# rpl-cmu/bevrender

Measured on AMD Instinct MI355X. Metric: samples/sec fwd+bwd, 6-cam 256x704 BEV-lift+corr, higher is better.
Workload: dtype bf16; 1 GPU; cfg3: 6-cam 256x704 features (64x64x176), 200x200 BEV, C=64 h=2 D=5, L=2 encoder layers (TSA+SCA), T=2 (1 no-grad history frame(s) + 1 fwd+bwd), correlation head with contrastive + lifted-structure losses, AdamW; batch 8 per GPU; backbone/render CNN excluded; global_batch=8, per_gpu_batch=8, parallelism=dp1

## Files before the change

bevrender_amd/_lib.py:

```python
from __future__ import annotations

import ctypes as C
import os
import subprocess
import threading

import torch

_HERE = os.path.dirname(os.path.abspath(__file__))
LIB_PATH = os.environ.get("BEVRENDER_LIB") or os.path.join(_HERE, "lib", "libbevrender_hip.so")
CSRC = os.path.join(_HERE, "csrc")

PREC_F32, PREC_BF16, PREC_F16, PREC_BF16X3 = 0, 1, 2, 3
ABI_VERSION = 6

SYMBOLS = [
    "bevr_abi_version", "bevr_strerror", "bevr_attn_table_dims", "bevr_attn_key_ws_bytes", "bevr_attn_key_prep",
    "bevr_attn_fwd", "bevr_attn_bwd_q",
    "bevr_attn_bwd_k", "bevr_attn_fwd_dropout", "bevr_attn_bwd_q_dropout", "bevr_attn_bwd_k_dropout", "bevr_attn_cell_fwd", "bevr_attn_cell_bwd_q", "bevr_attn_cell_bwd_k", "bevr_attn_tap_ws_bytes", "bevr_attn_tap_prep", "bevr_attn_tap_fwd", "bevr_attn_tap_bwd_q", "bevr_attn_tap_bwd_k", "bevr_attn_tap_fwd_dropout", "bevr_attn_tap_bwd_q_dropout", "bevr_attn_tap_bwd_k_dropout", "bevr_attn_gather_fwd", "bevr_attn_gather_fwd_rows", "bevr_attn_gather_fwd_x3", "bevr_attn_slab_ws_bytes", "bevr_attn_slab_prep", "bevr_attn_slab_bwd_q", "bevr_attn_slab_rows_ws_bytes", "bevr_attn_slab_rows_prep", "bevr_attn_slab_bwd_q_rows", "bevr_sample_fwd", "bevr_sample_bwd", "bevr_sample_fwd_bf16", "bevr_sample_bwd_bf16", "bevr_project_bev_grid", "bevr_project_bev_grid_masked", "bevr_corr_fwd",
    "bevr_corr_bwd", "bevr_recall_rank", "bevr_dwconv_fwd", "bevr_dwconv_bwd_w", "bevr_dwconv_res_gelu", "bevr_affine_warp_fwd", "bevr_affine_warp_bwd",
    "bevr_attn_bwd_k_ws_bytes", "bevr_attn_bwd_k_ws", "bevr_attn_tap_bwd_k_ws_bytes", "bevr_attn_tap_bwd_k_ws",
    "bevr_attn_slab_x3_ws_bytes", "bevr_attn_slab_x3_prep", "bevr_attn_slab_bwd_q_x3",
    "bevr_attn_tap_fwd_x3_dropout", "bevr_attn_tap_bwd_q_x3_dropout", "bevr_attn_tap_bwd_k_x3_dropout",
    "bevr_offset_head_fwd", "bevr_offset_head_bwd", "bevr_key_positions_fwd", "bevr_key_positions_bwd", "bevr_kv_project", "bevr_layernorm_fwd", "bevr_layernorm_bwd", "bevr_merge_views_fwd", "bevr_merge_views_bwd", "bevr_merge_tap_fwd", "bevr_merge_tap_bwd", "bevr_attn_bwd_prep", "bevr_pack_kv", "bevr_unpack_dkv",
]


class AttnDesc(C.Structure):
    _fields_ = [(n, C.c_int32) for n in (
        "n_prob", "q_div", "heads", "groups", "S", "Sp", "N", "Np", "Ht", "Wt", "Hp", "Wp",
        "y_off", "x_off", "precision", "reserved")]


class BevrError(RuntimeError):
    pass


_lib = None
_lock = threading.Lock()


def build(verbose: bool = False) -> str:
    cmd = ["make", "-C", CSRC, "-j", "4"]
    res = subprocess.run(cmd, capture_output=True, text=True)
    if verbose or res.returncode != 0:
        print(res.stdout)
        print(res.stderr)
# ... 57 lines not shown
        L.bevr_attn_slab_rows_prep.argtypes = [dp, fp, fp, vp, vp, vp]
        L.bevr_attn_slab_bwd_q_rows.argtypes = [dp, vp, vp, vp, vp, fp, vp, fp, fp, fp, fp, fp, ip, ip, vp]
        L.bevr_attn_slab_x3_ws_bytes.argtypes = [dp]
        L.bevr_attn_slab_x3_prep.argtypes = [dp, fp, fp, vp, vp, vp]
        L.bevr_attn_slab_bwd_q_x3.argtypes = [dp, vp, vp, vp, vp, fp, vp, fp, fp, fp, fp, fp, vp]
        L.bevr_sample_fwd.argtypes = [fp, fp, fp] + [ip] * 5 + [vp]
        L.bevr_sample_bwd.argtypes = [fp] * 5 + [ip] * 5 + [vp]
        L.bevr_sample_fwd_bf16.argtypes = [vp, fp, fp] + [ip] * 5 + [vp]
        L.bevr_sample_bwd_bf16.argtypes = [vp] + [fp] * 4 + [ip] * 5 + [vp]
        L.bevr_project_bev_grid.argtypes = [fp] * 4 + [ip] * 4 + [vp]
        L.bevr_project_bev_grid_masked.argtypes = [fp] * 4 + [ip] * 4 + [vp] + [ip] * 3 + [vp]
        L.bevr_corr_fwd.argtypes = [fp] * 5 + [ip] * 4 + [vp]
        L.bevr_corr_bwd.argtypes = [fp] * 8 + [ip] * 4 + [vp]
        L.bevr_recall_rank.argtypes = [fp, vp, ip, vp]
        L.bevr_dwconv_fwd.argtypes = [fp, fp, fp, fp] + [ip] * 7 + [vp]
        L.bevr_dwconv_bwd_w.argtypes = [fp, fp, fp, fp] + [ip] * 6 + [vp]
        L.bevr_dwconv_res_gelu.argtypes = [fp] * 5 + [ip] * 6 + [vp]
        L.bevr_affine_warp_fwd.argtypes = [fp, fp, fp] + [ip] * 4 + [vp]
        L.bevr_affine_warp_bwd.argtypes = [fp, fp, fp] + [ip] * 4 + [vp]
        L.bevr_offset_head_fwd.argtypes = [fp] * 7 + [C.c_longlong] + [ip] * 4 + [C.c_float, vp]
        L.bevr_offset_head_bwd.argtypes = [fp] * 13 + [C.c_longlong] + [ip] * 4 + [C.c_float, vp]
        L.bevr_layernorm_fwd.argtypes = [fp] * 6 + [C.c_longlong, ip, C.c_float, vp]
        L.bevr_layernorm_bwd.argtypes = [fp] * 8 + [C.c_longlong, ip, vp]
        L.bevr_kv_project.argtypes = [vp, ip, fp, C.c_longlong, vp, fp] + [ip] * 9 + [vp] * 6 + [ip, vp]
        L.bevr_key_positions_fwd.argtypes = [fp, fp, vp, fp] + [ip] * 8 + [C.c_float, C.c_float, vp]
        L.bevr_key_positions_bwd.argtypes = [fp, fp, vp, fp, fp] + [ip] * 8 + [C.c_float, C.c_float, vp]
        L.bevr_pack_kv.argtypes = [fp, fp, C.c_longlong, C.c_longlong] + [ip] * 6 + [vp] * 5
        L.bevr_merge_views_fwd.argtypes = [fp] * 5 + [ip] * 6 + [vp]
        L.bevr_merge_views_bwd.argtypes = [fp] * 9 + [ip] * 6 + [vp]
        L.bevr_merge_tap_fwd.argtypes = [fp] * 7 + [ip] * 6 + [vp]
        L.bevr_merge_tap_bwd.argtypes = [fp] * 13 + [ip] * 6 + [vp]
        L.bevr_attn_bwd_prep.argtypes = [fp] * 5 + [vp, vp, fp, fp] + [ip] * 3 + [vp]
        L.bevr_unpack_dkv.argtypes = [fp] * 4 + [C.c_longlong, C.c_longlong] + [ip] * 5 + [vp]
        for name in SYMBOLS:
            fn = getattr(L, name)
            if name in ("bevr_attn_key_ws_bytes", "bevr_attn_tap_ws_bytes", "bevr_attn_slab_ws_bytes",
                        "bevr_attn_slab_rows_ws_bytes", "bevr_attn_slab_x3_ws_bytes", "bevr_attn_bwd_k_ws_bytes", "bevr_attn_tap_bwd_k_ws_bytes"):
                fn.restype = C.c_size_t
            elif name not in ("bevr_strerror",):
                fn.restype = C.c_int
        if L.bevr_abi_version() != ABI_VERSION:
            raise BevrError(f"libbevrender_hip.so ABI version {L.bevr_abi_version()} != {ABI_VERSION}: rebuild "
                            "(make -C bevrender_amd/csrc)")
        _lib = L
    return _lib

# ... 6 lines not shown
```

bevrender_amd/csrc/dwconv.hip:

```cpp
#include "bevr_common.h"

namespace {

struct DwGeom {
  int B, H, W, C, k;
  long sb, sy, sx, sc;
  int nhwc;
};

__global__ __launch_bounds__(256) void dwconv_fwd_kernel(DwGeom g, const float* __restrict__ x, const float* __restrict__ w,
                                                         const float* __restrict__ bias, float* __restrict__ y, int flip) {
  const long n = (long)g.B * g.H * g.W * g.C;
  const long idx = (long)blockIdx.x * 256 + threadIdx.x;
  if (idx >= n) return;
  int c, xx, yy, b;
  if (g.nhwc) { c = idx % g.C; long t = idx / g.C; xx = t % g.W; t /= g.W; yy = t % g.H; b = t / g.H; }
  else { xx = idx % g.W; long t = idx / g.W; yy = t % g.H; t /= g.H; c = t % g.C; b = t / g.C; }
  const int p = g.k / 2;
  const float* wc = w + (long)c * g.k * g.k;
  const float* xb = x + b * g.sb + c * g.sc;
  float acc = bias ? bias[c] : 0.f;
  for (int dy = 0; dy < g.k; ++dy) {
    const int iy = yy + dy - p;
    if (iy < 0 || iy >= g.H) continue;
// ... 232 lines not shown
  }
  const DwGeom g = make_geom(B, H, W, C, k, nhwc);
  const long n = (long)B * H * W * C;
  hipLaunchKernelGGL(dwconv_fwd_kernel, dim3((unsigned)((n + 255) / 256)), dim3(256), 0, (hipStream_t)stream, g, x, w, bias, y,
                     flip);
  return (int)hipGetLastError();
}

extern "C" int bevr_dwconv_res_gelu(const float* x, const float* w, const float* bias, const float* aux, float* y, int B, int H,
                                    int W, int C, int k, int mode, void* stream) {
  if (!x || !w || !y || (mode == 2 && !aux)) return BEVR_E_NULL;
  if (B <= 0 || H <= 0 || W <= 0 || C <= 0 || (C & 3) || k != 3 || mode < 1 || mode > 3) return BEVR_E_SHAPE;
  if (!bevr_aligned16(x) || !bevr_aligned16(y) || (bias && !bevr_aligned16(bias)) || (aux && !bevr_aligned16(aux)))
    return BEVR_E_ALIGN;
  const long nthr = (long)B * H * ((W + DW_XT - 1) / DW_XT) * (C >> 2);
  const dim3 grid((unsigned)((nthr + 255) / 256));
  hipStream_t st = (hipStream_t)stream;
  if (mode == 1)
    hipLaunchKernelGGL((dwconv_fwd_nhwc4_kernel<3, 1>), grid, dim3(256), 0, st, B, H, W, C, x, w, bias, aux, y, 0);
  else if (mode == 2)
    hipLaunchKernelGGL((dwconv_fwd_nhwc4_kernel<3, 2>), grid, dim3(256), 0, st, B, H, W, C, x, w, bias, aux, y, 0);
  else
    hipLaunchKernelGGL((dwconv_fwd_nhwc4_kernel<3, 3>), grid, dim3(256), 0, st, B, H, W, C, x, w, (const float*)nullptr, aux, y, 1);
  return (int)hipGetLastError();
}

constexpr int DW_BANDS = 4;
__global__ __launch_bounds__(256) void dwconv_bwd_w_nchw3_kernel(int H, int W, const float* __restrict__ x,
                                                                const float* __restrict__ dy_, float* __restrict__ dw,
                                                                float* __restrict__ dbias, int C) {
  __shared__ float red[4][10];
  const int plane = blockIdx.x, band = blockIdx.y, xx = threadIdx.x;
  const int c = plane % C;
  const int rows = (H + DW_BANDS - 1) / DW_BANDS, y0 = band * rows, y1 = min(H, y0 + rows);
  const float* xp = x + (size_t)plane * H * W;
  const float* dp = dy_ + (size_t)plane * H * W;
  const bool on = xx < W;
  auto row3 = [&](int yy, float (&r)[3]) {
    const bool ry = on && yy >= 0 && yy < H;
    r[0] = (ry && xx >= 1) ? xp[(size_t)yy * W + xx - 1] : 0.f;
    r[1] = ry ? xp[(size_t)yy * W + xx] : 0.f;
    r[2] = (ry && xx + 1 < W) ? xp[(size_t)yy * W + xx + 1] : 0.f;
  };
  float acc[9] = {0.f, 0.f, 0.f, 0.f, 0.f, 0.f, 0.f, 0.f, 0.f}, accb = 0.f;
  float ra[3], rb[3], rc[3];
  row3(y0 - 1, ra);
// ... 53 lines not shown
```

bevrender_amd/model/SCA.py:

```python
import os

import torch
import torch.nn as nn

from .. import ops
from .SCA_deform_attn import SCADeformableAttention


MIN_CELL_KEYS = int(os.environ.get("BEVR_CELL_MIN", "1024"))


def pillar_grid(bev_bound, S: int, D: int, z_shift: float) -> torch.Tensor:
    X, Y, Z = float(bev_bound["X"]), float(bev_bound["Y"]), float(bev_bound["Z"])
    xs, ys, zs = X / S, Y / S, Z / D

    def bins(start, end, step, n):
        v = torch.arange(start, end, step)
        if v.numel() < n:
            raise ValueError("BEV bound / shape produce too few bins")
        return v[:n]

    gx = bins(0 + xs, X + xs, 2 * xs, S // 2)
    gy = bins(-Y + ys, Y + ys, 2 * ys, S)
    gz = bins(-Z + zs + z_shift, Z + zs + z_shift, 2 * zs, D)
# ... 18 lines not shown
            batch_size=batch_size, n_views=n_views, attn_drop_rate=attn_drop_rate, proj_drop_rate=proj_drop_rate,
            data_type=data_type, logger=logger, precision=precision)

    def sample_3d_points(self) -> torch.Tensor:
        return pillar_grid(self.bev_bound, self.bev_feat_shape, self.bev_depth_dim, self.z_shift)

    @property
    def points_2d_dict(self):
        return self.projector.bev_grid_to_camera(self.sample_3d_points())

    def reference_points(self, vehicle_code: int, device):
        key = (int(vehicle_code), str(device))
        if key not in self._ref_cache:
            pts = self.projector.bev_grid_to_camera(self.sample_3d_points(), device=device)[int(vehicle_code)]
            r = torch.stack(pts, 0)
            V, _, h, w, d = r.shape
            ref = r.permute(0, 2, 3, 4, 1).reshape(V, h, w * d, 2).contiguous()
            S, D = self.bev_feat_shape, self.bev_depth_dim
            yx = ref.reshape(V, -1, 2)[..., (1, 0)].double().cpu().numpy()
            order, split = ops.split_key_order(yx, S, 2 * S * D - 1, MIN_CELL_KEYS)
            self._ref_cache[key] = (ref, order.to(device), split)
        return self._ref_cache[key]

    def forward(self, query, img_feat, vehicle_type_idx, wandb_log_dict, return_wandb_log=True):
        B = query.shape[0]
        code = int(vehicle_type_idx) if not torch.is_tensor(vehicle_type_idx) else self._code(vehicle_type_idx)
        ref, order, split = self.reference_points(code, query.device)
        ref = ref[None].expand(B, -1, -1, -1, -1)
        if img_feat.dim() == 4:
            img_feat = img_feat.reshape(B, self.num_views, *img_feat.shape[1:])
        return self.spatial_deform_attn(x=img_feat, query=query, reference_points=ref,
                                        wandb_log_dict=wandb_log_dict, return_wandb_log=return_wandb_log,
                                        key_order=order, cell_split=split, split_is_pinned=True)

    def _code(self, t: torch.Tensor) -> int:
        codes = self.projector.vehicle_codes()
        if len(codes) == 1:
            return codes[0]
        return int(t.item())
```

bevrender_amd/model/SCA_deform_attn.py:

```python
import os

import torch
import torch.nn.functional as F
from torch import nn

from .. import ops, resolve_precision
from .model_utils import LayerNormProxy, attention_dropout, trunc_normal_

CELL_TAIL = int(os.environ.get("BEVR_CELL_TAIL", "128"))


class SCADeformableAttention(nn.Module):
    def __init__(self, bev_feat_shape, bev_depth_dim, dim_embed, n_heads, n_groups, stride, kernel_size,
                 scale_offset_range, batch_size, n_views=3, attn_drop_rate=0.0, proj_drop_rate=0.0,
                 data_type=torch.float32, logger=None, precision=None):
        super().__init__()
        self.n_channel_per_head = dim_embed // n_heads
        self.scale = self.n_channel_per_head ** -0.5
        self.n_heads = n_heads
        self.embed_dim = self.n_channel_per_head * n_heads
        self.n_groups = n_groups
        self.n_channel_per_group = self.embed_dim // n_groups
        self.n_heads_per_group = n_heads // n_groups
        self.query_height = self.query_width = bev_feat_shape
# ... 56 lines not shown
                rng = off.new_tensor([1.0 / (Hk - 1.0), 1.0 / (Wk - 1.0)]).reshape(1, 2, 1, 1)
                off = off.tanh() * rng * self.offset_range_factor
            pos = off.permute(0, 2, 3, 1).reshape(B, g, Hk, Wk, 2) + ref[:, v, None]
            if not self.scale_offset_range:
                pos = pos.clamp(-1.0, 1.0)
            outs.append(pos.reshape(B, g, Hk * Wk, 2))
        pos = torch.stack(outs, 1)
        if key_order is not None:
            N = Hk * Wk
            pos = pos.gather(3, key_order[None, :, None, :, None].expand(B, V, g, N, 2))
        return pos

    def _pinned_keys_tap(self, S, Hi, Wi):
        if not (self.scale_offset_range and ops.tap_supported(self.precision, self.n_groups)):
            return False
        Hk, Wk = S // 2, S * self.bev_depth_dim
        if Hk < 2 or Wk < 2:
            return False
        ymax = 0.5 * self.offset_range_factor / (Hk - 1.0) * (Hi - 1)
        xmax = 0.5 * self.offset_range_factor / (Wk - 1.0) * (Wi - 1)
        return (ymax < ops.TAP_R - 1 - 1e-3 or Hi <= ops.TAP_R) and (xmax < ops.TAP_C - 1 - 1e-3 or Wi <= ops.TAP_C)

    def forward(self, x, query, reference_points, wandb_log_dict, return_wandb_log=True, key_order=None,
                cell_split=None, split_is_pinned=False):
        B, V, C, Hi, Wi = x.shape
        S = query.shape[-1]
        if V != self.n_views:
            raise ValueError(f"expected {self.n_views} views, got {V}")
        g = self.n_groups
        pos = self.key_positions(query, reference_points.to(query.dtype), key_order)
        N = pos.shape[3]
        pos = pos.reshape(B * V * g, N, 2)
        drop = attention_dropout(self)
        Wt = self.rpe_table.shape[-1]
        pinned = split_is_pinned and self._pinned_keys_tap(S, Hi, Wi)
        if not (cell_split is not None and cell_split < N and g == 1):
            cell_split = None
        source = "kv"
        if x.is_cuda and ops.kv_source_supported(C, self.n_heads, g, self.precision):
            source = "kv_source"
        elif (x.is_cuda and pinned and cell_split is not None and self.precision == ops._lib.PREC_BF16X3
              and (drop is None or ops.tap_supported(self.precision, g, dropout=True))):
            source = "tap_pix"
        tap_source = False
        if cell_split is not None:
            route = ops.attention_route(self.precision, g, S, Wt, N, cell_split, "pinned" if pinned and source != "kv" else False,
                                        drop is not None, source, C, self.n_heads)
# ... 3 lines not shown
            n_tail = min(CELL_TAIL, max(0, N - cell_split - 1024))
            with torch.no_grad():
                a, b = ops.key_coords(pos[:, cell_split:], S, Wt, N - cell_split)
                dyn = ops.cell_order(a, b, n_tail)
            pos = torch.cat((pos[:, :cell_split], pos[:, cell_split:].gather(1, dyn[..., None].expand(-1, -1, 2))), 1)
            cell_split = cell_split + n_tail
        Wkv = torch.cat((self.proj_k.weight.flatten(1), self.proj_v.weight.flatten(1)), 0)
        bkv = torch.cat((self.proj_k.bias, self.proj_v.bias), 0)
        xf = x.reshape(B * V, C, Hi, Wi)
        if source == "kv_source":
            feat = (xf if xf.dtype == torch.bfloat16 else xf.float()).permute(0, 2, 3, 1).contiguous()
            src = dict(kv_source=(feat, Wkv, bkv))
        elif source == "tap_pix":
            xs = ops.sample_features(xf, pos[:, :cell_split].contiguous(), g)
            src = dict(kv=F.linear(xs, Wkv, bkv), tap_pix=(xf.permute(0, 2, 3, 1), Wkv, bkv))
        else:
            xs = ops.sample_features(xf, pos, g)
            src = dict(kv=F.linear(xs, Wkv, bkv))
        o = ops.attention_core(query, None, None, pos, self.rpe_table, heads=self.n_heads, groups=g, views=V,
                               precision=self.precision, cell_split=cell_split, tap_source=tap_source, attn_drop=drop,
                               concat_views=True, **src)
        out = ops.linear_rows(o, self.proj_out.weight.flatten(1), self.proj_out.bias)
        out = F.dropout(out, self.proj_drop_rate, self.training)
        return out.permute(0, 2, 1).reshape(B, C, S, S), wandb_log_dict
```

bevrender_amd/model/TSA.py:

```python
import torch
import torch.nn as nn

from .TSA_deform_attn import TSADeformableAttention


class TemporalSelfAttn(nn.Module):
    def __init__(self, bev_feat_shape, dim_embed, n_heads, n_groups, stride, kernel_size, batch_size,
                 scale_offset_range, n_views=3, attn_drop_rate=0.0, proj_drop_rate=0.0, data_type=torch.float32,
                 logger=None, precision=None):
        super().__init__()
        self.logger = logger
        assert n_heads % n_groups == 0, "n_heads must be divisible by n_groups"
        self.temporal_deform_attn = TSADeformableAttention(
            bev_feat_shape=bev_feat_shape, dim_embed=dim_embed, n_heads=n_heads, n_groups=n_groups, stride=stride,
            kernel_size=kernel_size, scale_offset_range=scale_offset_range, batch_size=batch_size, n_views=n_views,
            attn_drop_rate=attn_drop_rate, proj_drop_rate=proj_drop_rate, data_type=data_type, logger=logger,
            precision=precision)

    def forward(self, query, prev_bev, wandb_log_dict, return_wandb_log=True):
        return self.temporal_deform_attn(x=prev_bev, query=query, wandb_log_dict=wandb_log_dict,
                                         return_wandb_log=return_wandb_log)
```

bevrender_amd/model/TSA_deform_attn.py:

```python
import torch
import torch.nn.functional as F
from torch import nn

from .. import ops, resolve_precision
from .model_utils import (LayerNormProxy, attention_dropout, _dw_ok, depthwise_conv2d, depthwise_conv2d_nhwc, normalized_grid,
                          trunc_normal_)


class TSADeformableAttention(nn.Module):
    def __init__(self, bev_feat_shape, dim_embed, n_heads, n_groups, stride, kernel_size, scale_offset_range,
                 batch_size, n_views=3, attn_drop_rate=0.0, proj_drop_rate=0.0, data_type=torch.float32,
                 logger=None, precision=None):
        super().__init__()
        self.n_channel_per_head = dim_embed // n_heads
        self.scale = self.n_channel_per_head ** -0.5
        self.n_heads = n_heads
        self.embed_dim = self.n_channel_per_head * n_heads
        self.n_groups = n_groups
        self.n_channel_per_group = self.embed_dim // n_groups
        self.n_heads_per_group = n_heads // n_groups
        self.bev_h = self.bev_w = bev_feat_shape
        self.batch_size = batch_size
        self.scale_offset_range = scale_offset_range
        self.kernel_size, self.stride, self.n_views = kernel_size, stride, n_views
# ... 41 lines not shown
                                  co[3].weight.flatten(1), 1, co[1].norm.eps).permute(0, 3, 1, 2)
        else:
            y = co[2](co[1](z))
            off = F.linear(y.permute(0, 2, 3, 1), co[3].weight.flatten(1)).permute(0, 3, 1, 2)
        Hk, Wk = off.shape[-2:]
        if off.is_cuda and Hk > 1 and Wk > 1:
            fac = self.offset_range_factor if self.scale_offset_range else 1.0
            grid = normalized_grid(Hk, Wk, torch.float32, off.device).reshape(1, Hk * Wk, 2)
            pos = ops.key_positions(off.permute(0, 2, 3, 1).reshape(1, B * g, Hk * Wk, 2), grid,
                                    self._key_order(Hk, Wk, off.device)[None], B, g, sca_SD=None,
                                    use_tanh=bool(self.scale_offset_range), sy=fac / (Hk - 1.0), sx=fac / (Wk - 1.0))
            return pos.reshape(B * g, Hk * Wk, 2)
        if self.scale_offset_range:
            rng = off.new_tensor([1.0 / (Hk - 1.0), 1.0 / (Wk - 1.0)]).reshape(1, 2, 1, 1)
            off = off.tanh() * rng * self.offset_range_factor
        pos = off.permute(0, 2, 3, 1) + normalized_grid(Hk, Wk, off.dtype, off.device)[None]
        if not self.scale_offset_range:
            pos = pos.clamp(-1.0, 1.0)
        pos = pos.reshape(B * g, Hk * Wk, 2)
        if Hk > 1 and Wk > 1:
            pos = pos.index_select(1, self._key_order(Hk, Wk, pos.device))
        return pos

    def forward(self, x, query, wandb_log_dict, return_wandb_log=True):
        if x is None:
            x = query
        B, C, H, W = x.shape
        pos = self.key_positions(query)
        Wkv = torch.cat((self.proj_k.weight.flatten(1), self.proj_v.weight.flatten(1)), 0)
        bkv = torch.cat((self.proj_k.bias, self.proj_v.bias), 0)
        drop = attention_dropout(self)
        if x.is_cuda and ops.kv_source_supported(C, self.n_heads, self.n_groups, self.precision):
            feat = (x if x.dtype == torch.bfloat16 else x.float()).permute(0, 2, 3, 1).contiguous()
            o = ops.attention_core(query, None, None, pos, self.rpe_table, heads=self.n_heads, groups=self.n_groups,
                                   views=1, precision=self.precision, kv_source=(feat, Wkv, bkv), attn_drop=drop)
        else:
            xs = ops.sample_features(x, pos, self.n_groups)
            kv = F.linear(xs, Wkv, bkv)
            o = ops.attention_core(query, None, None, pos, self.rpe_table, heads=self.n_heads, groups=self.n_groups,
                                   views=1, precision=self.precision, kv=kv, attn_drop=drop)
        out = ops.linear_rows(o, self.proj_out.weight.flatten(1), self.proj_out.bias)
        out = F.dropout(out, self.proj_drop_rate, self.training)
        out = out.permute(0, 2, 1).reshape(B, C, H, W)
        return out, wandb_log_dict
```

bevrender_amd/model/encoder.py:

```python
import math

import torch
import torch.nn as nn
import torch.nn.functional as F

from .SCA import SpatialCrossAttn
from .TSA import TemporalSelfAttn
from .feedforward import FeedForwardLayer
from .img_backbone import PatchProjection, ResNet18_wo_fpn
from .model_utils import LayerNormProxy, TransformerMLPWithConv, depthwise_conv2d


class DropPath(nn.Module):

    def __init__(self, drop_prob=0.0):
        super().__init__()
        self.drop_prob = drop_prob

    def forward(self, x):
        if self.drop_prob == 0.0 or not self.training:
            return x
        keep = 1.0 - self.drop_prob
        mask = x.new_empty((x.shape[0],) + (1,) * (x.dim() - 1)).bernoulli_(keep)
        return x * mask / keep


class EncoderLayer(nn.Module):
    def __init__(self, bev_bound, bev2cmr_projector, n_views, bev_feat_shape, bev_depth_dim, z_shift, dim_embed,
                 expansion, stage_idx, n_groups, n_heads, stride, kernel_size, batch_size, scale_offset_range,
                 attn_drop_rate=0.0, proj_drop_rate=0.0, mlp_drop_rate=0.0, drop_path_rate=0.2, ffn_drop_rate=0.1,
                 data_type=torch.float32, logger=None, precision=None):
        super().__init__()
        self.logger, self.stage_idx, self.bev_feat_shape = logger, stage_idx, bev_feat_shape
# ... 1 lines not shown
        self.layer_scale = nn.Identity()
        self.layer_norm = LayerNormProxy(C)
        self.tsa_mlp = TransformerMLPWithConv(C, expansion, mlp_drop_rate)
        self.sca_mlp = TransformerMLPWithConv(C, expansion, mlp_drop_rate)
        self.drop_path = DropPath(drop_path_rate) if drop_path_rate > 0.0 else nn.Identity()
        self.tsa_local_percept_unit = nn.Conv2d(C, C, 3, 1, 1, groups=C)
        self.sca_local_percept_unit = nn.Conv2d(C, C, 3, 1, 1, groups=C)
        self.down_proj = nn.Sequential(nn.Conv2d(C, 2 * C, 3, 2, 1, bias=False), LayerNormProxy(2 * C))
        self.ffn_tsa = FeedForwardLayer(in_dim=bev_feat_shape, hidden_dim=C, dropout=ffn_drop_rate)
        self.ffn_sca = FeedForwardLayer(in_dim=bev_feat_shape, hidden_dim=C, dropout=ffn_drop_rate)
        common = dict(bev_feat_shape=bev_feat_shape, dim_embed=C, n_heads=n_heads, n_groups=n_groups, stride=stride,
                      kernel_size=kernel_size, batch_size=batch_size, scale_offset_range=scale_offset_range,
                      n_views=n_views, attn_drop_rate=attn_drop_rate, proj_drop_rate=proj_drop_rate,
                      data_type=data_type, logger=logger, precision=precision)
        self.temporal_self_attn = TemporalSelfAttn(**common)
        self.spatial_cross_attn = SpatialCrossAttn(bev_bound=bev_bound, bev2cmr_projector=bev2cmr_projector,
                                                   bev_depth_dim=bev_depth_dim, z_shift=z_shift, **common)

    def forward(self, bev_query, img_tensor, prev_bev, vehicle_pose, vehicle_type_idx, wandb_log_dict,
                return_wandb_log=True):
        x = bev_query
        if prev_bev is not None and not self.training:
            prev_bev = self.project_history_bev_feat(prev_bev, vehicle_pose)
        x = x + depthwise_conv2d(x, self.tsa_local_percept_unit)
        a, wandb_log_dict = self.temporal_self_attn(query=self.layer_norm(x), prev_bev=prev_bev,
                                                    wandb_log_dict=wandb_log_dict, return_wandb_log=return_wandb_log)
        x = self.drop_path(self.layer_scale(a)) + x
        x = self.drop_path(self.layer_scale(self.tsa_mlp(self.layer_norm(x)))) + x
        x = x + depthwise_conv2d(x, self.sca_local_percept_unit)
        a, wandb_log_dict = self.spatial_cross_attn(query=self.layer_norm(x), img_feat=img_tensor,
                                                    vehicle_type_idx=vehicle_type_idx, wandb_log_dict=wandb_log_dict,
                                                    return_wandb_log=return_wandb_log)
        x = self.drop_path(self.layer_scale(a)) + x
        x = self.drop_path(self.layer_scale(self.sca_mlp(self.layer_norm(x)))) + x
        return x, wandb_log_dict

    def project_history_bev_feat(self, bev, vehicle_pose, return_mask=False):
        from .. import ops
        pose = vehicle_pose.to(bev.device, torch.float32)
        prev_rot, curr_rot = pose[:, 0, 2], pose[:, 1, 2]
        delta = (pose[:, 0] - pose[:, 1])[:, :2]
        out = ops.affine_warp(bev, prev_rot, delta)
        out = ops.affine_warp(out, -curr_rot, torch.zeros_like(delta))
        if return_mask:
            return out, out != 0
        return out


class BEVEncoderStage(nn.Module):
    def __init__(self, bev_bound, bev2cmr_projector, batch_size, scale_offset_range, stage_idx=0, n_views=3,
                 expansion=4, dims=(64, 128), bev_feat_shapes=(56, 28), bev_depth_dim=5, z_shift=-1.0, depth=2,
                 n_heads=2, strides=8, n_groups=1, kernel_size=9, drop_rate=0.0, attn_drop_rate=0.0,
                 drop_path_rate=0.2, data_type=torch.float32, logger=None, precision=None):
        super().__init__()
        self.logger = logger
        dims, shapes = list(dims), list(bev_feat_shapes)
        self.curr_feat_dim, self.next_feat_dim = dims if len(dims) == 2 else (dims[0], dims[0])
        self.curr_bev_feat_shape, self.next_bev_feat_shape = shapes if len(shapes) == 2 else (shapes[0], shapes[0])
# ... 83 lines not shown
```

bevrender_amd/model/model_utils.py:

```python
import torch
import torch.nn.functional as F
from torch import nn


def _dw_ok(x, conv: nn.Conv2d) -> bool:
    k = conv.kernel_size[0]
    return (conv.groups == conv.in_channels == conv.out_channels and conv.stride == (1, 1)
            and conv.kernel_size == (k, k) and conv.padding == (k // 2, k // 2) and conv.dilation == (1, 1)
            and k % 2 == 1 and k <= 5 and x.dtype == torch.float32)


def depthwise_conv2d(x, conv: nn.Conv2d):
    if not x.is_cuda or not _dw_ok(x, conv):
        return conv(x)
    from .. import ops
    return ops.depthwise_conv(x, conv.weight, conv.bias, nhwc=False)


def depthwise_conv2d_nhwc(x, conv: nn.Conv2d):
    if not x.is_cuda or not _dw_ok(x, conv):
        return conv(x.permute(0, 3, 1, 2)).permute(0, 2, 3, 1)
    from .. import ops
    return ops.depthwise_conv(x, conv.weight, conv.bias, nhwc=True)

# ... 12 lines not shown
    def forward(self, x):
        xh = x.permute(0, 2, 3, 1)
        if x.is_cuda and x.dtype == torch.float32 and self.norm.elementwise_affine:
            from .. import ops
            if ops.layer_norm_supported(xh.shape[-1]):
                return ops.layer_norm(xh, self.norm.weight, self.norm.bias, self.norm.eps).permute(0, 3, 1, 2)
        y = F.layer_norm(xh, self.norm.normalized_shape, self.norm.weight, self.norm.bias, self.norm.eps)
        return y.permute(0, 3, 1, 2)


class TransformerMLPWithConv(nn.Module):

    def __init__(self, channels, expansion, drop):
        super().__init__()
        self.dim1, self.dim2 = channels, channels * expansion
        self.linear1 = nn.Sequential(nn.Conv2d(self.dim1, self.dim2, 1, 1, 0))
        self.drop1 = nn.Dropout(drop)
        self.act = nn.GELU()
        self.linear2 = nn.Sequential(nn.Conv2d(self.dim2, self.dim1, 1, 1, 0))
        self.drop2 = nn.Dropout(drop)
        self.dwc = nn.Conv2d(self.dim2, self.dim2, 3, 1, 1, groups=self.dim2)

    def forward(self, x):
        xh = x.permute(0, 2, 3, 1)
        y = self.drop1(pointwise_conv_nhwc(xh, self.linear1[0]))
        from .. import ops
        if isinstance(self.act, nn.GELU) and self.act.approximate == "none" and ops.dwconv_res_gelu_supported(y, self.dwc.weight) \
                and _dw_ok(y, self.dwc):
            y = ops.dwconv_res_gelu(y, self.dwc.weight, self.dwc.bias)
        else:
            y = self.act(y + depthwise_conv2d_nhwc(y, self.dwc))
        y = self.drop2(pointwise_conv_nhwc(y, self.linear2[0]))
        return y.permute(0, 3, 1, 2)


class LayerScale(nn.Module):
    def __init__(self, dim: int, inplace: bool = False, init_values: float = 1e-5):
        super().__init__()
        self.inplace = inplace
        self.weight = nn.Parameter(torch.full((dim,), init_values))

    def forward(self, x):
        w = self.weight.view(-1, 1, 1)
        return x.mul_(w) if self.inplace else x * w


def normalized_grid(H: int, W: int, dtype, device) -> torch.Tensor:
    gy = torch.arange(H, dtype=dtype, device=device) / (H - 1.0) * 2.0 - 1.0
    gx = torch.arange(W, dtype=dtype, device=device) / (W - 1.0) * 2.0 - 1.0
    return torch.stack(torch.meshgrid(gy, gx, indexing="ij"), -1)


def trunc_normal_(t: torch.Tensor, std: float = 1.0):
    return nn.init.trunc_normal_(t, std=std)


# ... 6 lines not shown
```

bevrender_amd/ops.py:

```python
from __future__ import annotations

import ctypes as C
import math
import os
from dataclasses import dataclass, replace as dc_replace
from types import SimpleNamespace
from typing import Optional, Tuple

import torch
import torch.nn.functional as F

from . import _lib

LOG2E = 1.4426950408889634
HEAD_DIM = 32


def perm32(r: int) -> int:
    return (r & ~12) | ((r & 4) << 1) | ((r & 8) >> 1)


_PERM_CACHE = {}


# ... 1337 lines not shown

    @staticmethod
    def backward(ctx, dy):
        x, gamma, mean, rstd = ctx.saved_tensors
        Cc = x.shape[-1]
        dy = dy.float().contiguous()
        dx = torch.empty_like(x)
        dg = torch.zeros(Cc, device=x.device, dtype=torch.float32)
        db = torch.zeros_like(dg)
        _launch("bevr_layernorm_bwd", _ptr(x), _ptr(gamma), _ptr(dy), _ptr(mean), _ptr(rstd), _ptr(dx), _ptr(dg), _ptr(db),
                x.numel() // Cc, Cc, _stream())
        return dx, dg, db, None


def layer_norm_supported(C: int) -> bool:
    c4 = C // 4
    return C % 4 == 0 and 0 < c4 <= 64 and (c4 & (c4 - 1)) == 0


def layer_norm(x: torch.Tensor, gamma: torch.Tensor, beta: torch.Tensor, eps: float = 1e-5) -> torch.Tensor:
    return _LayerNorm.apply(x, gamma, beta, eps)


class _KeyPositions(torch.autograd.Function):

    @staticmethod
    def forward(ctx, off, ref, order, B, G, sca_SD, use_tanh, sy, sx):
        _require_gpu(off, ref, order)
        off, ref = off.float().contiguous(), ref.float().contiguous()
        V, P = off.shape[0], off.shape[1]
        N = ref.shape[1]
        S, D = sca_SD if sca_SD else (0, 0)
        order = None if order is None else order.to(torch.int32).contiguous()
        pos = torch.empty(B, V, G, N, 2, device=off.device, dtype=torch.float32)
        ctx.args = (V, P, G, N, 1 if sca_SD else 0, S, D, 1 if use_tanh else 0, float(sy), float(sx))
        _launch("bevr_key_positions_fwd", _ptr(off), _ptr(ref), _ptr(order), _ptr(pos), *ctx.args, _stream())
        ctx.save_for_backward(off, ref, order)
        return pos

    @staticmethod
    def backward(ctx, dpos):
        off, ref, order = ctx.saved_tensors
        doff = torch.empty_like(off)
        _launch("bevr_key_positions_bwd", _ptr(off), _ptr(ref), _ptr(order), _ptr(dpos.float().contiguous()), _ptr(doff),
                *ctx.args, _stream())
        return doff, None, None, None, None, None, None, None, None
# ... 122 lines not shown
```

include/bevrender_hip.h:

```cpp
#ifndef BEVRENDER_HIP_H
#define BEVRENDER_HIP_H

#include <stddef.h>
#include <stdint.h>

#ifdef __cplusplus
extern "C" {
#endif

#define BEVR_ABI_VERSION 6

enum {
  BEVR_OK = 0,
  BEVR_E_NULL = -1,
  BEVR_E_SHAPE = -2,
  BEVR_E_PRECISION = -3,
  BEVR_E_ALIGN = -4
};

enum { BEVR_PREC_F32 = 0, BEVR_PREC_BF16 = 1, BEVR_PREC_F16 = 2, BEVR_PREC_BF16X3 = 3 };

int bevr_abi_version(void);
const char* bevr_strerror(int code);

// ... 145 lines not shown
                  int n, int m, int E, int normalize, void* stream);
int bevr_corr_bwd(const float* cam, const float* map, const float* D, const float* dD,
                  const float* inv_norm_cam, const float* inv_norm_map, float* dcam, float* dmap,
                  int n, int m, int E, int normalize, void* stream);
int bevr_recall_rank(const float* D, int32_t* rank, int n, void* stream);

int bevr_dwconv_fwd(const float* x, const float* w, const float* bias, float* y,
                    int B, int H, int W, int C, int k, int nhwc, int flip, void* stream);
int bevr_dwconv_bwd_w(const float* x, const float* dy, float* dw, float* dbias,
                      int B, int H, int W, int C, int k, int nhwc, void* stream);
int bevr_dwconv_res_gelu(const float* x, const float* w, const float* bias, const float* aux, float* y, int B, int H, int W,
                         int C, int k, int mode, void* stream);

int bevr_pack_kv(const float* k, const float* v, long long ld, long long pstride, int n_prob, int N, int Np, int heads,
                 int c, int precision, void* Kr, void* Vr, void* Kt, void* Vt, void* stream);
int bevr_unpack_dkv(const float* dK, const float* dV, float* dk, float* dv, long long ld, long long pstride, int n_prob,
                    int N, int Np, int heads, int c, void* stream);

int bevr_layernorm_fwd(const float* x, const float* gamma, const float* beta, float* y, float* mean, float* rstd,
                       long long rows, int C, float eps, void* stream);
int bevr_layernorm_bwd(const float* x, const float* gamma, const float* dy, const float* mean, const float* rstd,
                       float* dx, float* dgamma, float* dbeta, long long rows, int C, void* stream);

int bevr_merge_views_fwd(const float* O_r, const float* L_r, const float* O_c, const float* L_c, float* out, int n_prob,
                         int views, int heads, int S, int Sp, int c, void* stream);
int bevr_merge_views_bwd(const float* dout, const float* O_r, const float* L_r, const float* O_c, const float* L_c,
                         float* dO_r, float* dL_r, float* dO_c, float* dL_c, int n_prob, int views, int heads, int S,
                         int Sp, int c, void* stream);
int bevr_merge_tap_fwd(const float* O_r, const float* L_r, const float* Rn, const float* L_c, const float* Vp, const float* bv,
                       float* out, int n_prob, int views, int heads, int S, int Sp, int c, void* stream);
int bevr_merge_tap_bwd(const float* dout, const float* O_r, const float* L_r, const float* Rn, const float* L_c, const float* Vp,
                       const float* bv, float* dO_r, float* dL_r, float* dRn, float* dL_c, float* dVp, float* dbv, int n_prob,
                       int views, int heads, int S, int Sp, int c, void* stream);

int bevr_attn_bwd_prep(const float* dO, const float* O, const float* scale, const float* dLSE, const float* LSE0, void* dOe,
                       void* dOt, float* delta, float* stats, int n_ph, int Mp, int precision, void* stream);

int bevr_kv_project(const void* feat, int feat_bf16, const float* pos, long long pos_pstride, const void* Wkv,
                    const float* bkv, int nb, int Hi, int Wi, int C, int N, int Np, int heads, int c, int precision,
                    void* Kr, void* Vr, void* Kt, void* Vt, float* vnorm2_max, float* knorm2_max, int groups,
                    void* stream);

int bevr_key_positions_fwd(const float* off, const float* ref, const int* order, float* pos, int V, int P, int G, int N,
                           int sca, int S, int D, int use_tanh, float sy, float sx, void* stream);
int bevr_key_positions_bwd(const float* off, const float* ref, const int* order, const float* dpos, float* doff, int V,
                           int P, int G, int N, int sca, int S, int D, int use_tanh, float sy, float sx, void* stream);
// ... 17 lines not shown
```

Baseline: 5.908 samples/s.

## Fuse residual add with LayerNorm and keep encoder layer in NHWC rows

Adds fused add+LayerNorm forward/backward kernels and a dwconv+residual kernel, and gives the encoder layer a row-major (NHWC) path. TSA/SCA/MLP outputs stay in rows layout instead of being permuted to NCHW and back. The aim is to cut elementwise kernel launches and layout copies between the attention blocks. The path is gated by an env flag and shape checks, and dgamma/dbeta are accumulated with atomics across slots.

```diff
diff --git a/bevrender_amd/_lib.py b/bevrender_amd/_lib.py
--- a/bevrender_amd/_lib.py
+++ b/bevrender_amd/_lib.py
@@ -23,6 +23,7 @@
     "bevr_attn_slab_x3_ws_bytes", "bevr_attn_slab_x3_prep", "bevr_attn_slab_bwd_q_x3",
     "bevr_attn_tap_fwd_x3_dropout", "bevr_attn_tap_bwd_q_x3_dropout", "bevr_attn_tap_bwd_k_x3_dropout",
     "bevr_offset_head_fwd", "bevr_offset_head_bwd", "bevr_key_positions_fwd", "bevr_key_positions_bwd", "bevr_kv_project", "bevr_layernorm_fwd", "bevr_layernorm_bwd", "bevr_merge_views_fwd", "bevr_merge_views_bwd", "bevr_merge_tap_fwd", "bevr_merge_tap_bwd", "bevr_attn_bwd_prep", "bevr_pack_kv", "bevr_unpack_dkv",
+    "bevr_add_ln_fwd", "bevr_add_ln_bwd", "bevr_dwconv_res",
 ]
 
 
@@ -126,6 +127,9 @@
         L.bevr_offset_head_bwd.argtypes = [fp] * 13 + [C.c_longlong] + [ip] * 4 + [C.c_float, vp]
         L.bevr_layernorm_fwd.argtypes = [fp] * 6 + [C.c_longlong, ip, C.c_float, vp]
         L.bevr_layernorm_bwd.argtypes = [fp] * 8 + [C.c_longlong, ip, vp]
+        L.bevr_add_ln_fwd.argtypes = [fp] * 8 + [C.c_longlong, ip, C.c_float, vp]
+        L.bevr_add_ln_bwd.argtypes = [fp] * 9 + [ip, C.c_longlong, ip, vp]
+        L.bevr_dwconv_res.argtypes = [fp] * 4 + [ip] * 6 + [vp]
         L.bevr_kv_project.argtypes = [vp, ip, fp, C.c_longlong, vp, fp] + [ip] * 9 + [vp] * 6 + [ip, vp]
         L.bevr_key_positions_fwd.argtypes = [fp, fp, vp, fp] + [ip] * 8 + [C.c_float, C.c_float, vp]
         L.bevr_key_positions_bwd.argtypes = [fp, fp, vp, fp, fp] + [ip] * 8 + [C.c_float, C.c_float, vp]
diff --git a/bevrender_amd/csrc/dwconv.hip b/bevrender_amd/csrc/dwconv.hip
--- a/bevrender_amd/csrc/dwconv.hip
+++ b/bevrender_amd/csrc/dwconv.hip
@@ -278,6 +278,17 @@
     hipLaunchKernelGGL((dwconv_fwd_nhwc4_kernel<3, 2>), grid, dim3(256), 0, st, B, H, W, C, x, w, bias, aux, y, 0);
   else
     hipLaunchKernelGGL((dwconv_fwd_nhwc4_kernel<3, 3>), grid, dim3(256), 0, st, B, H, W, C, x, w, (const float*)nullptr, aux, y, 1);
+  return (int)hipGetLastError();
+}
+
+extern "C" int bevr_dwconv_res(const float* x, const float* w, const float* bias, float* y, int B, int H, int W, int C, int k,
+                               int flip, void* stream) {
+  if (!x || !w || !y) return BEVR_E_NULL;
+  if (B <= 0 || H <= 0 || W <= 0 || C <= 0 || (C & 3) || k != 3 || flip < 0 || flip > 1) return BEVR_E_SHAPE;
+  if (!bevr_aligned16(x) || !bevr_aligned16(y) || (bias && !bevr_aligned16(bias))) return BEVR_E_ALIGN;
+  const long nthr = (long)B * H * ((W + DW_XT - 1) / DW_XT) * (C >> 2);
+  hipLaunchKernelGGL((dwconv_fwd_nhwc4_kernel<3, 3>), dim3((unsigned)((nthr + 255) / 256)), dim3(256), 0, (hipStream_t)stream, B,
+                     H, W, C, x, w, bias, (const float*)nullptr, y, flip);
   return (int)hipGetLastError();
 }
 
diff --git a/bevrender_amd/csrc/layer_glue.hip b/bevrender_amd/csrc/layer_glue.hip
--- /dev/null
+++ b/bevrender_amd/csrc/layer_glue.hip
@@ -0,0 +1,128 @@
+#include "bevr_common.h"
+
+namespace {
+
+constexpr int GL_THREADS = 256;
+
+__device__ __forceinline__ float group_sum(float v, int c4n) {
+  for (int sh = c4n >> 1; sh > 0; sh >>= 1) v += __shfl_xor(v, sh);
+  return v;
+}
+
+__global__ __launch_bounds__(GL_THREADS) void add_ln_fwd_kernel(const float* __restrict__ a, const float* __restrict__ x,
+                                                                const float* __restrict__ gamma, const float* __restrict__ beta,
+                                                                float* __restrict__ x1, float* __restrict__ n,
+                                                                float* __restrict__ mean, float* __restrict__ rstd,
+                                                                long long rows, int C, float eps) {
+  const int c4n = C >> 2, c4 = threadIdx.x % c4n, slots = GL_THREADS / c4n;
+  const f32x4 g4 = *reinterpret_cast<const f32x4*>(gamma + c4 * 4), b4 = *reinterpret_cast<const f32x4*>(beta + c4 * 4);
+  const float inv_c = 1.0f / (float)C;
+  const long long n_it = (rows + (long long)gridDim.x * slots - 1) / ((long long)gridDim.x * slots);
+  for (long long it = 0; it < n_it; ++it) {
+    const long long row = (it * gridDim.x + blockIdx.x) * slots + threadIdx.x / c4n;
+    const bool live = row < rows;
+    const long long off = (live ? row : 0) * C + c4 * 4;
+    f32x4 v = *reinterpret_cast<const f32x4*>(x + off);
+    if (a) v = *reinterpret_cast<const f32x4*>(a + off) + v;
+    const float mu = group_sum(v[0] + v[1] + v[2] + v[3], c4n) * inv_c;
+    const f32x4 d = v - f32x4{mu, mu, mu, mu};
+    const float var = group_sum(d[0] * d[0] + d[1] * d[1] + d[2] * d[2] + d[3] * d[3], c4n) * inv_c;
+    const float rs = rsqrtf(var + eps);
+    if (live) {
+      if (a) *reinterpret_cast<f32x4*>(x1 + off) = v;
+      *reinterpret_cast<f32x4*>(n + off) = d * rs * g4 + b4;
+      if (c4 == 0) {
+        mean[row] = mu;
+        rstd[row] = rs;
+      }
+    }
+  }
+}
+
+__global__ __launch_bounds__(GL_THREADS) void add_ln_bwd_kernel(const float* __restrict__ x1, const float* __restrict__ gamma,
+                                                                const float* __restrict__ dn, const float* __restrict__ dx1,
+                                                                const float* __restrict__ mean, const float* __restrict__ rstd,
+                                                                float* __restrict__ g_out, float* __restrict__ dgamma,
+                                                                float* __restrict__ dbeta, int n_slots, long long rows, int C) {
+  __shared__ f32x4 red[2][GL_THREADS];
+  const int c4n = C >> 2, c4 = threadIdx.x % c4n, slots = GL_THREADS / c4n;
+  const f32x4 g4 = *reinterpret_cast<const f32x4*>(gamma + c4 * 4);
+  const float inv_c = 1.0f / (float)C;
+  f32x4 ag = {0.f, 0.f, 0.f, 0.f}, ab = {0.f, 0.f, 0.f, 0.f};
+  const long long n_it = (rows + (long long)gridDim.x * slots - 1) / ((long long)gridDim.x * slots);
+  for (long long it = 0; it < n_it; ++it) {
+    const long long row = (it * gridDim.x + blockIdx.x) * slots + threadIdx.x / c4n;
+    const bool live = row < rows;
+    const long long r0 = live ? row : 0;
+    const long long off = r0 * C + c4 * 4;
+    const f32x4 v = *reinterpret_cast<const f32x4*>(x1 + off);
+    f32x4 g = *reinterpret_cast<const f32x4*>(dn + off);
+    if (!live) g = f32x4{0.f, 0.f, 0.f, 0.f};
+    const float mu = mean[r0], rs = rstd[r0];
+    const f32x4 xh = (v - f32x4{mu, mu, mu, mu}) * rs;
+    const f32x4 gg = g * g4;
+    const float m1 = group_sum(gg[0] + gg[1] + gg[2] + gg[3], c4n) * inv_c;
+    const float m2 = group_sum(gg[0] * xh[0] + gg[1] * xh[1] + gg[2] * xh[2] + gg[3] * xh[3], c4n) * inv_c;
+    if (live) {
+      f32x4 o = (gg - f32x4{m1, m1, m1, m1} - xh * m2) * rs;
+      if (dx1) o = *reinterpret_cast<const f32x4*>(dx1 + off) + o;
+      *reinterpret_cast<f32x4*>(g_out + off) = o;
+    }
+    ag += g * xh;
+    ab += g;
+  }
+  red[0][threadIdx.x] = ag;
+  red[1][threadIdx.x] = ab;
+  __syncthreads();
+  for (int u = threadIdx.x; u < 2 * c4n; u += GL_THREADS) {
+    const int which = u / c4n, q = u % c4n;
+    f32x4 s = {0.f, 0.f, 0.f, 0.f};
+    for (int sl = 0; sl < slots; ++sl) s += red[which][sl * c4n + q];
+    float* dst = (which ? dbeta : dgamma) + (size_t)(blockIdx.x % n_slots) * C + q * 4;
+#pragma unroll
+    for (int k = 0; k < 4; ++k) atomicAdd(dst + k, s[k]);
+  }
+}
+
+int check(long long rows, int C) {
+  const int c4n = C >> 2;
+  if (rows <= 0 || C <= 0 || (C & 3) || c4n > 64 || (c4n & (c4n - 1))) return BEVR_E_SHAPE;
+  return BEVR_OK;
+}
+
+int grid_of(long long rows, int C) {
+  const long long per = GL_THREADS / (C >> 2);
+  long long g = (rows + per - 1) / per;
+  if (g > 256 * 8) g = 256 * 8;
+  return (int)(g < 1 ? 1 : g);
+}
+
+}
+
+extern "C" int bevr_add_ln_fwd(const float* a, const float* x, const float* gamma, const float* beta, float* x1, float* n,
+                               float* mean, float* rstd, long long rows, int C, float eps, void* stream) {
+  if (!x || !gamma || !beta || !n || !mean || !rstd || (a && !x1)) return BEVR_E_NULL;
+  int rc = check(rows, C);
+  if (rc) return rc;
+  if (!bevr_aligned16(x) || !bevr_aligned16(n) || !bevr_aligned16(gamma) || !bevr_aligned16(beta) ||
+      (a && (!bevr_aligned16(a) || !bevr_aligned16(x1))))
+    return BEVR_E_ALIGN;
+  hipLaunchKernelGGL(add_ln_fwd_kernel, dim3(grid_of(rows, C)), dim3(GL_THREADS), 0, (hipStream_t)stream, a, x, gamma, beta, x1,
+                     n, mean, rstd, rows, C, eps);
+  return (int)hipGetLastError();
+}
+
+extern "C" int bevr_add_ln_bwd(const float* x1, const float* gamma, const float* dn, const float* dx1, const float* mean,
+                               const float* rstd, float* g, float* dgamma, float* dbeta, int n_slots, long long rows, int C,
+                               void* stream) {
+  if (!x1 || !gamma || !dn || !mean || !rstd || !g || !dgamma || !dbeta) return BEVR_E_NULL;
+  int rc = check(rows, C);
+  if (rc) return rc;
+  if (n_slots < 1 || n_slots > 256) return BEVR_E_SHAPE;
+  if (!bevr_aligned16(x1) || !bevr_aligned16(dn) || !bevr_aligned16(g) || !bevr_aligned16(gamma) ||
+      (dx1 && !bevr_aligned16(dx1)))
+    return BEVR_E_ALIGN;
+  hipLaunchKernelGGL(add_ln_bwd_kernel, dim3(grid_of(rows, C)), dim3(GL_THREADS), 0, (hipStream_t)stream, x1, gamma, dn, dx1,
+                     mean, rstd, g, dgamma, dbeta, n_slots, rows, C);
+  return (int)hipGetLastError();
+}
diff --git a/bevrender_amd/model/SCA.py b/bevrender_amd/model/SCA.py
--- a/bevrender_amd/model/SCA.py
+++ b/bevrender_amd/model/SCA.py
@@ -64,7 +64,7 @@
             self._ref_cache[key] = (ref, order.to(device), split)
         return self._ref_cache[key]
 
-    def forward(self, query, img_feat, vehicle_type_idx, wandb_log_dict, return_wandb_log=True):
+    def forward(self, query, img_feat, vehicle_type_idx, wandb_log_dict, return_wandb_log=True, rows=False):
         B = query.shape[0]
         code = int(vehicle_type_idx) if not torch.is_tensor(vehicle_type_idx) else self._code(vehicle_type_idx)
         ref, order, split = self.reference_points(code, query.device)
@@ -73,7 +73,7 @@
             img_feat = img_feat.reshape(B, self.num_views, *img_feat.shape[1:])
         return self.spatial_deform_attn(x=img_feat, query=query, reference_points=ref,
                                         wandb_log_dict=wandb_log_dict, return_wandb_log=return_wandb_log,
-                                        key_order=order, cell_split=split, split_is_pinned=True)
+                                        key_order=order, cell_split=split, split_is_pinned=True, rows=rows)
 
     def _code(self, t: torch.Tensor) -> int:
         codes = self.projector.vehicle_codes()
diff --git a/bevrender_amd/model/SCA_deform_attn.py b/bevrender_amd/model/SCA_deform_attn.py
--- a/bevrender_amd/model/SCA_deform_attn.py
+++ b/bevrender_amd/model/SCA_deform_attn.py
@@ -102,7 +102,7 @@
         return (ymax < ops.TAP_R - 1 - 1e-3 or Hi <= ops.TAP_R) and (xmax < ops.TAP_C - 1 - 1e-3 or Wi <= ops.TAP_C)
 
     def forward(self, x, query, reference_points, wandb_log_dict, return_wandb_log=True, key_order=None,
-                cell_split=None, split_is_pinned=False):
+                cell_split=None, split_is_pinned=False, rows=False):
         B, V, C, Hi, Wi = x.shape
         S = query.shape[-1]
         if V != self.n_views:
@@ -152,4 +152,6 @@
                                concat_views=True, **src)
         out = ops.linear_rows(o, self.proj_out.weight.flatten(1), self.proj_out.bias)
         out = F.dropout(out, self.proj_drop_rate, self.training)
+        if rows:
+            return out.reshape(B, S, S, C), wandb_log_dict
         return out.permute(0, 2, 1).reshape(B, C, S, S), wandb_log_dict
diff --git a/bevrender_amd/model/TSA.py b/bevrender_amd/model/TSA.py
--- a/bevrender_amd/model/TSA.py
+++ b/bevrender_amd/model/TSA.py
@@ -17,6 +17,6 @@
             attn_drop_rate=attn_drop_rate, proj_drop_rate=proj_drop_rate, data_type=data_type, logger=logger,
             precision=precision)
 
-    def forward(self, query, prev_bev, wandb_log_dict, return_wandb_log=True):
+    def forward(self, query, prev_bev, wandb_log_dict, return_wandb_log=True, rows=False):
         return self.temporal_deform_attn(x=prev_bev, query=query, wandb_log_dict=wandb_log_dict,
-                                         return_wandb_log=return_wandb_log)
+                                         return_wandb_log=return_wandb_log, rows=rows)
diff --git a/bevrender_amd/model/TSA_deform_attn.py b/bevrender_amd/model/TSA_deform_attn.py
--- a/bevrender_amd/model/TSA_deform_attn.py
+++ b/bevrender_amd/model/TSA_deform_attn.py
@@ -87,7 +87,7 @@
             pos = pos.index_select(1, self._key_order(Hk, Wk, pos.device))
         return pos
 
-    def forward(self, x, query, wandb_log_dict, return_wandb_log=True):
+    def forward(self, x, query, wandb_log_dict, return_wandb_log=True, rows=False):
         if x is None:
             x = query
         B, C, H, W = x.shape
@@ -106,5 +106,7 @@
                                    views=1, precision=self.precision, kv=kv, attn_drop=drop)
         out = ops.linear_rows(o, self.proj_out.weight.flatten(1), self.proj_out.bias)
         out = F.dropout(out, self.proj_drop_rate, self.training)
+        if rows:
+            return out.reshape(B, H, W, C), wandb_log_dict
         out = out.permute(0, 2, 1).reshape(B, C, H, W)
         return out, wandb_log_dict
diff --git a/bevrender_amd/model/encoder.py b/bevrender_amd/model/encoder.py
--- a/bevrender_amd/model/encoder.py
+++ b/bevrender_amd/model/encoder.py
@@ -8,7 +8,7 @@
 from .TSA import TemporalSelfAttn
 from .feedforward import FeedForwardLayer
 from .img_backbone import PatchProjection, ResNet18_wo_fpn
-from .model_utils import LayerNormProxy, TransformerMLPWithConv, depthwise_conv2d
+from .model_utils import LayerNormProxy, TransformerMLPWithConv, _dw_ok, depthwise_conv2d
 
 
 class DropPath(nn.Module):
@@ -56,6 +56,8 @@
         x = bev_query
         if prev_bev is not None and not self.training:
             prev_bev = self.project_history_bev_feat(prev_bev, vehicle_pose)
+        if self._fused_ok(x):
+            return self._forward_rows(x, img_tensor, prev_bev, vehicle_type_idx, wandb_log_dict, return_wandb_log)
         x = x + depthwise_conv2d(x, self.tsa_local_percept_unit)
         a, wandb_log_dict = self.temporal_self_attn(query=self.layer_norm(x), prev_bev=prev_bev,
                                                     wandb_log_dict=wandb_log_dict, return_wandb_log=return_wandb_log)
@@ -68,6 +70,36 @@
         x = self.drop_path(self.layer_scale(a)) + x
         x = self.drop_path(self.layer_scale(self.sca_mlp(self.layer_norm(x)))) + x
         return x, wandb_log_dict
+
+    def _fused_ok(self, x):
+        from .. import ops
+        norm = self.layer_norm.norm
+        lpus = (self.tsa_local_percept_unit, self.sca_local_percept_unit)
+        drop_is_id = isinstance(self.drop_path, nn.Identity) or not self.training or self.drop_path.drop_prob == 0.0
+        return (x.is_cuda and x.dtype == torch.float32 and x.dim() == 4 and ops.fused_layer_enabled()
+                and norm.elementwise_affine and ops.layer_norm_supported(x.shape[1])
+                and all(_dw_ok(x, u) and u.kernel_size == (3, 3) for u in lpus)
+                and drop_is_id and isinstance(self.layer_scale, nn.Identity))
+
+    def _forward_rows(self, bev_query, img_tensor, prev_bev, vehicle_type_idx, wandb_log_dict, return_wandb_log):
+        from .. import ops
+        norm = self.layer_norm.norm
+        gamma, beta, eps = norm.weight, norm.bias, norm.eps
+        x = bev_query.permute(0, 2, 3, 1).contiguous()
+        tsa_u, sca_u = self.tsa_local_percept_unit, self.sca_local_percept_unit
+        x, n = ops.lpu_layer_norm(x, tsa_u.weight, tsa_u.bias, gamma, beta, eps)
+        a, wandb_log_dict = self.temporal_self_attn(query=n.permute(0, 3, 1, 2), prev_bev=prev_bev,
+                                                    wandb_log_dict=wandb_log_dict, return_wandb_log=return_wandb_log,
+                                                    rows=True)
+        x, n = ops.add_layer_norm(a, x, gamma, beta, eps)
+        x = self.tsa_mlp.forward_rows(n) + x
+        x, n = ops.lpu_layer_norm(x, sca_u.weight, sca_u.bias, gamma, beta, eps)
+        a, wandb_log_dict = self.spatial_cross_attn(query=n.permute(0, 3, 1, 2), img_feat=img_tensor,
+                                                    vehicle_type_idx=vehicle_type_idx, wandb_log_dict=wandb_log_dict,
+                                                    return_wandb_log=return_wandb_log, rows=True)
+        x, n = ops.add_layer_norm(a, x, gamma, beta, eps)
+        x = self.sca_mlp.forward_rows(n) + x
+        return x.permute(0, 3, 1, 2), wandb_log_dict
 
     def project_history_bev_feat(self, bev, vehicle_pose, return_mask=False):
         from .. import ops
diff --git a/bevrender_amd/model/model_utils.py b/bevrender_amd/model/model_utils.py
--- a/bevrender_amd/model/model_utils.py
+++ b/bevrender_amd/model/model_utils.py
@@ -58,7 +58,9 @@
         self.dwc = nn.Conv2d(self.dim2, self.dim2, 3, 1, 1, groups=self.dim2)
 
     def forward(self, x):
-        xh = x.permute(0, 2, 3, 1)
+        return self.forward_rows(x.permute(0, 2, 3, 1)).permute(0, 3, 1, 2)
+
+    def forward_rows(self, xh):
         y = self.drop1(pointwise_conv_nhwc(xh, self.linear1[0]))
         from .. import ops
         if isinstance(self.act, nn.GELU) and self.act.approximate == "none" and ops.dwconv_res_gelu_supported(y, self.dwc.weight) \
@@ -66,8 +68,7 @@
             y = ops.dwconv_res_gelu(y, self.dwc.weight, self.dwc.bias)
         else:
             y = self.act(y + depthwise_conv2d_nhwc(y, self.dwc))
-        y = self.drop2(pointwise_conv_nhwc(y, self.linear2[0]))
-        return y.permute(0, 3, 1, 2)
+        return self.drop2(pointwise_conv_nhwc(y, self.linear2[0]))
 
 
 class LayerScale(nn.Module):
diff --git a/bevrender_amd/ops.py b/bevrender_amd/ops.py
--- a/bevrender_amd/ops.py
+++ b/bevrender_amd/ops.py
@@ -1383,6 +1383,111 @@
     return _LayerNorm.apply(x, gamma, beta, eps)
 
 
+def fused_layer_enabled() -> bool:
+    return os.environ.get("BEVR_FUSED_LAYER", "1") != "0"
+
+
+ADD_LN_SLOTS = 32
+
+
+def _add_ln_bwd(x1, gamma, mean, rstd, dx1, dn):
+    Cc = x1.shape[-1]
+    if dn is None:
+        dg = torch.zeros(Cc, device=x1.device, dtype=torch.float32)
+        return dx1, dg, torch.zeros_like(dg)
+    dn = dn.float().contiguous()
+    dx1 = None if dx1 is None else dx1.float().contiguous()
+    g = torch.empty_like(x1)
+    dgb = torch.zeros(2, ADD_LN_SLOTS, Cc, device=x1.device, dtype=torch.float32)
+    _launch("bevr_add_ln_bwd", _ptr(x1), _ptr(gamma), _ptr(dn), _ptr(dx1), _ptr(mean), _ptr(rstd), _ptr(g), _ptr(dgb[0]),
+            _ptr(dgb[1]), ADD_LN_SLOTS, x1.numel() // Cc, Cc, _stream(), flops=0.0,
+            nbytes=float((4 if dx1 is not None else 3) * x1.numel() * 4))
+    dgb = dgb.sum(1)
+    return g, dgb[0], dgb[1]
+
+
+class _AddLN(torch.autograd.Function):
+
+    @staticmethod
+    def forward(ctx, a, x, gamma, beta, eps):
+        _require_gpu(a, x, gamma, beta)
+        a, x = a.float().contiguous(), x.float().contiguous()
+        gamma, beta = gamma.float().contiguous(), beta.float().contiguous()
+        Cc = x.shape[-1]
+        rows = x.numel() // Cc
+        x1, n = torch.empty_like(x), torch.empty_like(x)
+        mean = torch.empty(rows, device=x.device, dtype=torch.float32)
+        rstd = torch.empty_like(mean)
+        _launch("bevr_add_ln_fwd", _ptr(a), _ptr(x), _ptr(gamma), _ptr(beta), _ptr(x1), _ptr(n), _ptr(mean), _ptr(rstd), rows,
+                Cc, float(eps), _stream(), flops=0.0, nbytes=float(4 * x.numel() * 4))
+        ctx.save_for_backward(x1, gamma, mean, rstd)
+        ctx.set_materialize_grads(False)
+        return x1, n
+
+    @staticmethod
+    def backward(ctx, dx1, dn):
+        x1, gamma, mean, rstd = ctx.saved_tensors
+        g, dg, db = _add_ln_bwd(x1, gamma, mean, rstd, dx1, dn)
+        return g, g, dg, db, None
+
+
+def add_layer_norm(a: torch.Tensor, x: torch.Tensor, gamma: torch.Tensor, beta: torch.Tensor, eps: float = 1e-5):
+    if a.shape != x.shape:
+        raise ValueError(f"add_layer_norm: shapes {tuple(a.shape)} and {tuple(x.shape)} differ")
+    return _AddLN.apply(a, x, gamma, beta, eps)
+
+
+class _LpuLN(torch.autograd.Function):
+
+    @staticmethod
+    def forward(ctx, x, weight, bias, gamma, beta, eps):
+        _require_gpu(x, weight, bias, gamma, beta)
+        x, w = x.float().contiguous(), weight.float().contiguous()
+        b = None if bias is None else bias.float().contiguous()
+        gamma, beta = gamma.float().contiguous(), beta.float().contiguous()
+        B, H, W, Cc = x.shape
+        rows = B * H * W
+        x1, n = torch.empty_like(x), torch.empty_like(x)
+        mean = torch.empty(rows, device=x.device, dtype=torch.float32)
+        rstd = torch.empty_like(mean)
+        _launch("bevr_dwconv_res", _ptr(x), _ptr(w), _ptr(b), _ptr(x1), B, H, W, Cc, 3, 0, _stream(), flops=0.0,
+                nbytes=float(2 * x.numel() * 4))
+        _launch("bevr_add_ln_fwd", None, _ptr(x1), _ptr(gamma), _ptr(beta), None, _ptr(n), _ptr(mean), _ptr(rstd), rows, Cc,
+                float(eps), _stream(), flops=0.0, nbytes=float(2 * x.numel() * 4))
+        ctx.save_for_backward(x, w, x1, gamma, mean, rstd)
+        ctx.has_bias = b is not None
+        ctx.set_materialize_grads(False)
+        return x1, n
+
+    @staticmethod
+    def backward(ctx, dx1, dn):
+        x, w, x1, gamma, mean, rstd = ctx.saved_tensors
+        B, H, W, Cc = x.shape
+        g, dg, db = _add_ln_bwd(x1, gamma, mean, rstd, dx1, dn)
+        if g is None:
+            return None, None, None, dg, db, None
+        g = g.float().contiguous()
+        dx = dw = dbias = None
+        if ctx.needs_input_grad[0]:
+            dx = torch.empty_like(x)
+            _launch("bevr_dwconv_res", _ptr(g), _ptr(w), None, _ptr(dx), B, H, W, Cc, 3, 1, _stream(), flops=0.0,
+                    nbytes=float(2 * x.numel() * 4), label="bevr_dwconv_res(flip)")
+        if ctx.needs_input_grad[1] or (ctx.has_bias and ctx.needs_input_grad[2]):
+            dw = torch.zeros_like(w)
+            dbias = torch.zeros(Cc, device=x.device, dtype=torch.float32) if ctx.has_bias else None
+            _launch("bevr_dwconv_bwd_w", _ptr(x), _ptr(g), _ptr(dw), _ptr(dbias), B, H, W, Cc, 3, 1, _stream())
+        return dx, dw, dbias, dg, db, None
+
+
+def lpu_layer_norm_supported(x: torch.Tensor, weight: torch.Tensor) -> bool:
+    return (x.is_cuda and x.dtype == torch.float32 and x.dim() == 4 and layer_norm_supported(x.shape[-1])
+            and tuple(weight.shape) == (x.shape[-1], 1, 3, 3))
+
+
+def lpu_layer_norm(x: torch.Tensor, weight: torch.Tensor, bias, gamma: torch.Tensor, beta: torch.Tensor, eps: float = 1e-5):
+    return _LpuLN.apply(x, weight, bias, gamma, beta, eps)
+
+
 class _KeyPositions(torch.autograd.Function):
 
     @staticmethod
diff --git a/include/bevrender_hip.h b/include/bevrender_hip.h
--- a/include/bevrender_hip.h
+++ b/include/bevrender_hip.h
@@ -191,6 +191,14 @@
 int bevr_layernorm_bwd(const float* x, const float* gamma, const float* dy, const float* mean, const float* rstd,
                        float* dx, float* dgamma, float* dbeta, long long rows, int C, void* stream);
 
+int bevr_add_ln_fwd(const float* a, const float* x, const float* gamma, const float* beta, float* x1, float* n,
+                    float* mean, float* rstd, long long rows, int C, float eps, void* stream);
+int bevr_add_ln_bwd(const float* x1, const float* gamma, const float* dn, const float* dx1, const float* mean,
+                    const float* rstd, float* g, float* dgamma, float* dbeta, int n_slots, long long rows, int C,
+                    void* stream);
+int bevr_dwconv_res(const float* x, const float* w, const float* bias, float* y, int B, int H, int W, int C, int k,
+                    int flip, void* stream);
+
 int bevr_merge_views_fwd(const float* O_r, const float* L_r, const float* O_c, const float* L_c, float* out, int n_prob,
                          int views, int heads, int S, int Sp, int c, void* stream);
 int bevr_merge_views_bwd(const float* dout, const float* O_r, const float* L_r, const float* O_c, const float* L_c,
```

Result: no change. 5.942 samples/s, median of 6 (+0.6%).
